# joelle-o-world/dusp

Measured on AMD Instinct MI355X. Metric: rendered Msamples/sec (whole node) + HBM GB/s fraction, 1024-voice 48kHz, higher is better.
Workload: dtype f64; 1 GPU; configs[2] per-voice: 1024 voices/GPU x Multiply(Osc(10k), Ramp(T,1,0) triggered), 60s @48000 Hz, every voice's PCM written; voices_per_gpu=1024, voices_total=1024, n_samples=2880000, engine=fused, parallelism=voices sharded over 1 GPU(s), no collective

## Files before the change

### dusp_amd/csrc/device_util.hpp

```cpp
#pragma once
#if !defined(__HIPCC_RTC__)
#include <hip/hip_runtime.h>
#endif

#include "device_types.hpp"
#include "filter_lamda.hpp"

namespace dusp {
namespace {

__device__ __forceinline__ int lsb_exponent(double x) {
    int ex;
    const double fr = frexp(fabs(x), &ex);
    const long long m = (long long)ldexp(fr, 53);
    return ex - 53 + __builtin_ctzll((unsigned long long)m);
}
__device__ __forceinline__ uint64_t addmod(uint64_t a, uint64_t b, uint64_t S) {
    const uint64_t s = a + b;
    return s >= S ? s - S : s;
}
__device__ __forceinline__ uint64_t mulmod(uint64_t a, uint64_t n, uint64_t S) {
    uint64_t acc = 0;
    for (int bit = 63 - __builtin_clzll(n | 1); bit >= 0; --bit) {
        acc = addmod(acc, acc, S);
        if ((n >> bit) & 1) acc = addmod(acc, a, S);
    }
    return acc;
}

__device__ __forceinline__ float operand_value(const DevOperand &o, const float *params, uint32_t n_inst, uint32_t inst) {
    return o.kind == SRC_PARAM ? params[(size_t)o.idx * n_inst + inst] : o.cval;
}

enum : int { TABLE_FORM_DATA = 0, TABLE_FORM_SAW = 1, TABLE_FORM_SQUARE = 2, TABLE_FORM_TRIANGLE = 3, TABLE_FORM_8BIT = 4 };

#if defined(__HIPCC__) || defined(__HIPCC_RTC__)
#define DUSP_HD __host__ __device__ __forceinline__
#else
#define DUSP_HD inline
#endif

struct TableForm {
    int32_t form;
    uint32_t sr, half, quarter;
    double N, rcp_N, srd, rcp_sr;
};

DUSP_HD TableForm make_table_form(int form, uint32_t sample_rate) {
    TableForm F;
    F.form = form;
    F.sr = sample_rate;
    F.half = sample_rate / 2;
    F.quarter = sample_rate / 4;
    F.N = (double)sample_rate + 1.0;
    F.rcp_N = 1.0 / F.N;
    F.srd = (double)sample_rate;
    F.rcp_sr = 1.0 / F.srd;
    return F;
}

DUSP_HD double refined_quotient(double x, double d, double rcp) {
    const double q = x * rcp;
    return fma(fma(-q, d, x), rcp, q);
}

DUSP_HD double js_round_small(double x) {
    const double r = floor(x + 0.5);
    return (r == 0.0 && (x < 0.0 || (x == 0.0 && 1.0 / x < 0.0))) ? -0.0 : r;
}

DUSP_HD float closed_table_entry(const TableForm &F, uint32_t i) {
    if (F.form == TABLE_FORM_SQUARE) return i < F.half ? 1.f : -1.f;
    if (i >= F.sr) return 0.f;
    if (F.form == TABLE_FORM_SAW) return (float)(-1.0 + refined_quotient((double)(2u * i), F.N, F.rcp_N));
    const uint32_t seg = (i >= F.quarter ? 1u : 0u) + (i >= 2u * F.quarter ? 1u : 0u) + (i >= 3u * F.quarter ? 1u : 0u);
    const float base = (float)(refined_quotient((double)(i - seg * F.quarter), F.srd, F.rcp_sr) * 4.0);
    return seg == 0 ? base : seg == 1 ? (float)(1.0 - (double)base) : seg == 2 ? -base : (float)(-1.0 + (double)base);
}
DUSP_HD float eightbit_of_sine(float sine) { return (float)(js_round_small((double)sine * 128.0) / 128.0); }

__device__ __forceinline__ uint32_t abs_diff(uint32_t a, uint32_t b) {
    uint32_t r;
    asm("v_sad_u32 %0, %1, %2, 0" : "=v"(r) : "v"(a), "s"(b));
    return r;
}

template <int TBL>
struct Table {
    const float *g;
    const float *h;
    uint32_t N, M;
    TableForm form;
    __device__ __forceinline__ const float *word(uint32_t k) const {
        return (const float *)((const char *)h + ((k + (k >> 5)) << 2));
    }
    __device__ __forceinline__ float at(uint32_t i) const {
        if (TBL == 0) return g[i];
        if (TBL == 2) return closed_table_entry(form, i);
        const bool upper = i > M;
        const float v = *word(abs_diff(i, M) + (upper ? 0u : 1u));
        const float s = upper ? -v : v;
        return TBL == 3 ? eightbit_of_sine(s) : s;
    }
    __device__ __forceinline__ void pair(uint32_t i, float &a, float &b) const {
        if (TBL == 0) {
            a = g[i];
            b = g[i + 1];
            return;
        }
        if (TBL == 2) {
            a = closed_table_entry(form, i);
            b = closed_table_entry(form, i + 1 <= form.sr ? i + 1 : form.sr);
            return;
        }
        if (TBL == 3) {
            a = at(i);
            b = at(i + 1 < N ? i + 1 : N - 1);
            return;
        }
        const bool upper = i > M;
        const float *p = word(abs_diff(i, M));
        const float p0 = p[0], p1 = p[1];
        a = upper ? -p0 : p1;
        b = upper ? -p1 : p0;
    }
    template <bool D32>
    __device__ __forceinline__ void pair_delta_at(uint32_t a_img, bool upper, double &a, double &d) const {
        const float *p = word(a_img);
        const float p0 = p[0], p1 = p[1];
        a = (double)(upper ? -p0 : p1);
        delta<D32>(p0, p1, d);
    }
    template <bool D32>
    __device__ __forceinline__ void pair_delta(uint32_t i, double &a, double &d) const {
        if (TBL == 0) {
            const float x = g[i], y = g[i + 1];
            a = (double)x;
            delta<D32>(y, x, d);
        } else
            pair_delta_at<D32>(abs_diff(i, M), i > M, a, d);
    }
    template <bool D32>
    static __device__ __forceinline__ void delta(float y, float x, double &d) {
        if (D32) {
            float df;
            asm("v_sub_f32 %0, %1, %2" : "=v"(df) : "v"(y), "v"(x));
            d = (double)df;
        } else
            d = (double)y - (double)x;
    }
};

__device__ __forceinline__ float lerp_delta(double a, double d, uint32_t F) {
    return (float)fma(d, (double)F * (1.0 / 4294967296.0), a);
}

constexpr uint32_t kPhaseBias = 0x41300000u;
struct LeanPhase {
    template <bool WRAPPED>
    static __device__ __forceinline__ void locate(unsigned long long Pc, uint32_t sr, uint32_t M, uint32_t &a_img, bool &upper, double &fraction) {
        const uint32_t h = (uint32_t)(Pc >> 32);
        if (WRAPPED) {
            a_img = abs_diff(h, kPhaseBias + M);
            upper = h > kPhaseBias + M;
        } else {
            const uint32_t s = abs_diff(h, kPhaseBias + sr);
            a_img = abs_diff(s, M);
            upper = (s > M) != (h < kPhaseBias + sr);
        }
        fraction = __builtin_amdgcn_fract(__longlong_as_double((long long)Pc));
    }
    static __device__ __forceinline__ uint32_t index(unsigned long long Pc, uint32_t sr) {
        const uint32_t h = (uint32_t)(Pc >> 32);
        return min(h - kPhaseBias, h - (kPhaseBias + sr));
    }
    static __device__ __forceinline__ unsigned long long step(unsigned long long P, unsigned long long c, uint32_t sr) {
        const unsigned long long s = P + c;
        const uint32_t h = (uint32_t)(s >> 32);
        const uint32_t u = h - sr;
        return ((unsigned long long)(u >= kPhaseBias ? u : h) << 32) | (uint32_t)s;
    }
};

__device__ __forceinline__ uint32_t mod_u32(uint32_t x, uint32_t m, double inv_m) {
    const uint32_t q = (uint32_t)((double)x * inv_m);
    uint32_t r = x - q * m;
    if ((int32_t)r < 0) r += m;
    if (r >= m) r -= m;
    return r;
}
__device__ __forceinline__ uint64_t mod_u64(uint64_t x, uint64_t m, double inv_m) {
    const uint64_t q = (uint64_t)((double)x * inv_m);
    uint64_t r = x - q * m;
    if ((int64_t)r < 0) r += m;
    if ((int64_t)r < 0) r += m;
    if (r >= m) r -= m;
    if (r >= m) r -= m;
    return r;
}

__device__ __forceinline__ unsigned long long mod_u64_lifted(unsigned long long x, unsigned long long m, double inv_m) {
    return mod_u64(x, m, inv_m);
}

template <bool FINITE>
__device__ __forceinline__ float fix_out(float v) {
    if (FINITE) return v + 0.f;
    return __builtin_amdgcn_classf(v, 0x23) ? 0.f : v;
}

template <bool VEC>
__device__ __forceinline__ void store4(float *row, const float (&v)[4], uint64_t t, uint64_t n_samples) {
    if (VEC) {
#ifdef DUSP_NT_STORES
        __builtin_nontemporal_store(f32x4{v[0], v[1], v[2], v[3]}, (f32x4 *)row);
#else
        *(f32x4 *)row = f32x4{v[0], v[1], v[2], v[3]};
#endif
    } else
        for (int c = 0; c < 4; ++c)
            if (t + c < n_samples) row[c] = v[c];
}

template <int BLOCK>
__device__ __forceinline__ void load_half_table(float *lds, const float *table, uint32_t sample_rate) {
    const uint32_t last = sample_rate / 2 + 1;
    const uint32_t n_words = last + (last >> 5) + 2;
    for (uint32_t q = threadIdx.x; q < n_words; q += BLOCK) {
        const uint32_t t = (q / 33) * 32 + (q % 33);
        lds[q] = table[last - min(t, last)];
    }
    __syncthreads();
}

__host__ __device__ inline size_t half_table_lds_bytes(uint32_t sample_rate) { return (size_t)half_table_image_bytes(sample_rate); }

}
}
```

### dusp_amd/csrc/fused_engine.hip

```cpp
#include <hip/hip_runtime.h>

#include <type_traits>

#include "device_types.hpp"
#include "fused_device.hpp"
#include "fused_plan.hpp"
#include "repeat_add.hpp"

namespace dusp {

namespace {

template <bool FASTDIV>
__device__ __forceinline__ float ramp_value(const FusedArgs &A, double tn, double dy) {
    const double tt = fmin(tn, A.r_d);
    double q;
    if (FASTDIV) {
        q = tt * A.r_rcp;
        const double rem = fma(-q, A.r_d, tt);
        q = fma(rem, A.r_rcp, q);
    } else
        q = tt / A.r_d;
    return (float)(A.r_y0 + q * dy);
}

__device__ __forceinline__ float shape_value(const FusedArgs &A, double t, double srd) {
    const double l = (double)A.s_min, h = (double)A.s_max;
    if (t <= 0.0) return (float)((A.s_left_is_shape ? (double)A.s_table[0] : A.s_left) * (h - l) + l);
    if (t > srd) return (float)((A.s_right_is_shape ? (double)A.s_table[(uint32_t)srd] : A.s_right) * (h - l) + l);
    if (t != t) return __builtin_nanf("");
    const double fl = floor(t), frac = t - fl;
    return (float)(l + (h - l) * ((double)A.s_table[(int)ceil(t)] * frac + (double)A.s_table[(int)fl] * (1.0 - frac)));
}

__device__ __forceinline__ void start_phase(const OscRec &rc, uint32_t seg, uint32_t lane, uint64_t (&P)[4]) {
    const uint64_t base = addmod(addmod(rc.P0, rc.Fm, rc.S), mulmod(rc.segstep, seg, rc.S), rc.S);
    P[0] = addmod(base, mulmod(rc.step4, lane, rc.S), rc.S);
    for (int c = 1; c < 4; ++c) P[c] = addmod(P[c - 1], rc.Fm, rc.S);
}

}

__global__ void dusp_fused_prepare(FusedArgs A, OscRec *recs) {
    const uint32_t inst = blockIdx.x * blockDim.x + threadIdx.x;
    if (inst >= A.n_inst) return;
    const uint32_t sr = A.sample_rate;
    const double srd = (double)sr;
    OscRec rc;
    double fd = (double)operand_value(A.f, A.params, A.n_inst, inst);
    rc.bad = !(fabs(fd) <= 3.0e38);
    if (rc.bad) fd = 0.0;
    if (fabs(fd) >= srd) fd = fmod(fd, srd);
    int E = 0;
    if (fd != 0.0) E = min(E, lsb_exponent(fd));
    if (A.phase0 != 0.0) E = min(E, lsb_exponent(A.phase0));
    const int Emin = -(62 - (32 - __builtin_clz(sr)));
    if (E < Emin) E = Emin;
    rc.E = E;
    rc.u = ldexp(1.0, E);
    rc.S = (uint64_t)sr << (-E);
    const long long F = (long long)rint(ldexp(fd, -E));
    rc.Fm = F >= 0 ? (uint64_t)F : rc.S - (uint64_t)(-F);
    if (rc.Fm >= rc.S) rc.Fm -= rc.S;
    rc.P0 = (uint64_t)rint(ldexp(A.phase0, -E));
    if (rc.P0 >= rc.S) rc.P0 %= rc.S;
    rc.step4 = mulmod(rc.Fm, 4, rc.S);
    rc.step256 = mulmod(rc.Fm, kChunk, rc.S);
    rc.segstep = mulmod(rc.Fm, (uint64_t)A.seg_groups * kChunk, rc.S);
    rc.gain = A.gain.kind == SRC_PARAM || A.gain.kind == SRC_CONST ? operand_value(A.gain, A.params, A.n_inst, inst) : 1.f;
    rc.pad = 0;
    recs[inst] = rc;

    const uint64_t T_end = (uint64_t)A.n_chunks * kChunk;
    double phase_end = (double)addmod(rc.P0, mulmod(rc.Fm, T_end, rc.S), rc.S) * rc.u;
    if (rc.bad) phase_end = __builtin_nan("");
    A.end_state[(size_t)A.osc_state_word * A.n_inst + inst] = phase_end;
    if (A.ramp_state_word >= 0) {
        const double t_end = A.r_playing ? fmin(A.r_t0 + (double)T_end, A.r_d) : A.r_t0;
        const bool playing_end = A.r_playing && (A.r_t0 + (double)T_end <= A.r_d);
        A.end_state[(size_t)A.ramp_state_word * A.n_inst + inst] = t_end;
        A.end_state[(size_t)(A.ramp_state_word + 1) * A.n_inst + inst] = playing_end ? 1.0 : 0.0;
    }
    if (A.shape_state_word >= 0) {
        const double t_end = A.s_playing ? repeat_add(A.s_t0, A.s_c, T_end) : A.s_t0;
        A.end_state[(size_t)A.shape_state_word * A.n_inst + inst] = t_end;
        A.end_state[(size_t)(A.shape_state_word + 1) * A.n_inst + inst] = A.s_playing ? 1.0 : 0.0;
        A.end_state[(size_t)(A.shape_state_word + 2) * A.n_inst + inst] = (A.s_finished || (T_end > 0 && t_end > srd)) ? 1.0 : 0.0;
    }
}

template <int KIND, int TBL, int R, bool FASTDIV, bool FINITE, int BLOCK>
__global__ void __launch_bounds__(BLOCK) dusp_fused_kernel(FusedArgs A, const OscRec *__restrict__ recs) {
    extern __shared__ __attribute__((aligned(16))) float lds_table[];
    Table<TBL> table;
    table.g = A.table;
    table.h = lds_table;
    table.N = A.sample_rate + 1;
    table.M = A.sample_rate / 2;
    table.form = make_table_form(A.table_form, A.sample_rate);
    if (TBL == 1) load_half_table<BLOCK>(lds_table, A.table, A.sample_rate);
    const uint32_t lane = threadIdx.x & 63u;
    constexpr uint32_t waves_per_block = BLOCK / 64;
    constexpr int RS = R < 4 ? R : 4;
    const uint32_t n_blk = (A.n_inst + R - 1) / R;
    const uint64_t n_items = (uint64_t)n_blk * A.n_seg;
    const uint64_t total_waves = (uint64_t)gridDim.x * waves_per_block;
    const double srd = (double)A.sample_rate;
    const uint32_t sr = A.sample_rate;
    const double dy = A.r_y1 - A.r_y0;
    const uint32_t n_full = A.vec4_ok ? (uint32_t)(A.n_samples / kChunk) : 0u;

    for (uint64_t item = (uint64_t)blockIdx.x * waves_per_block + (threadIdx.x >> 6); item < n_items; item += total_waves) {
        const uint32_t blk = A.seg_major ? (uint32_t)(item / A.n_seg) : (uint32_t)(item % n_blk);
        const uint32_t seg = A.seg_major ? (uint32_t)(item % A.n_seg) : (uint32_t)(item / n_blk);
        const uint32_t g0 = seg * A.seg_groups;
        const uint32_t g1 = min(g0 + A.seg_groups, A.n_groups);
        const uint32_t gm = max(g0, min(g1, n_full));
        const uint64_t t_start = (uint64_t)g0 * kChunk;

        uint32_t inst[R];
        int e_min = 0;
        bool any_bad = false;
#pragma unroll
        for (int r = 0; r < R; ++r) {
            inst[r] = min(blk * R + r, A.n_inst - 1);
            e_min = min(e_min, recs[inst[r]].E);
            any_bad = any_bad || recs[inst[r]].bad;
        }
        float *const row0 = A.out + t_start + lane * 4;
        const double tn0 = A.r_t0 + (A.r_playing ? (double)(t_start + lane * 4 + 1) : 0.0);
        const double tn_step = A.r_playing ? (double)kChunk : 0.0;
        const double tn_c = A.r_playing ? 1.0 : 0.0;
        double tn;
        const double st0 = (KIND == FUSED_OSC_SHAPE && A.s_playing) ? repeat_add(A.s_t0, A.s_c, t_start) : A.s_t0;
        double st;
        auto ramp4 = [&](float (&rv)[4]) {
            if (KIND == FUSED_OSC_SHAPE) {
                if (!A.s_playing) {
#pragma unroll
                    for (int c = 0; c < 4; ++c) rv[c] = shape_value(A, st, srd);
                } else {
                    long long T, ce;
                    int K;
                    if (linear_run(st, A.s_c, kChunk, T, ce, K)) {
                        T += (long long)(lane * 4) * ce;
#pragma unroll
                        for (int c = 0; c < 4; ++c) {
                            T += ce;
                            rv[c] = shape_value(A, ldexp((double)T, K - 52), srd);
                        }
                        st = ldexp((double)(T + (long long)(kChunk - 4 - lane * 4) * ce), K - 52);
                    } else {
                        double t = repeat_add(st, A.s_c, (uint64_t)lane * 4);
#pragma unroll
                        for (int c = 0; c < 4; ++c) rv[c] = shape_value(A, t = t + A.s_c, srd);
                        st = __shfl(t, 63, 64);
                    }
                }
            }
            if (KIND == FUSED_OSC_RAMP) {
                rv[0] = ramp_value<FASTDIV>(A, tn, dy);
#pragma unroll
                for (int c = 1; c < 4; ++c) rv[c] = ramp_value<FASTDIV>(A, tn + tn_c * c, dy);
                tn += tn_step;
            }
        };
        auto finish = [&](float v, float rv, float gain) {
            if (KIND == FUSED_OSC_RAMP || KIND == FUSED_OSC_SHAPE) v = v * rv;
            if (KIND == FUSED_OSC_GAIN) v = v * gain;
            return fix_out<FINITE>(v);
        };

        if (e_min == 0 && !any_bad) {
            uint32_t idx[R][4], step[R];
            size_t roff[R];
            float gain[R];
#pragma unroll
            for (int r = 0; r < R; ++r) {
                const OscRec rc = recs[inst[r]];
                uint64_t P[4];
                start_phase(rc, seg, lane, P);
                for (int c = 0; c < 4; ++c) idx[r][c] = (uint32_t)P[c];
                step[r] = (uint32_t)rc.step256;
                roff[r] = (size_t)inst[r] * A.n_samples;
                gain[r] = rc.gain;
            }
            tn = tn0;
            st = st0;
            float *row = row0;
            auto run = [&](uint32_t ga, uint32_t gb, auto vec) {
                for (uint32_t g = ga; g < gb; ++g) {
                    float rv[4] = {1.f, 1.f, 1.f, 1.f};
                    ramp4(rv);
#pragma unroll
                    for (int r = 0; r < R; ++r) {
                        float v[4];
#pragma unroll
                        for (int c = 0; c < 4; ++c) {
                            v[c] = finish(table.at(idx[r][c]), rv[c], gain[r]);
                            idx[r][c] += step[r];
                            idx[r][c] = min(idx[r][c], idx[r][c] - sr);
                        }
                        store4<decltype(vec)::value>(row + roff[r], v, (uint64_t)g * kChunk + lane * 4, A.n_samples);
                    }
                    row += kChunk;
                }
            };
            run(g0, gm, std::true_type{});
            run(gm, g1, std::false_type{});
        } else if (e_min >= -32 && !any_bad && A.fx32_ok) {
            for (int sub = 0; sub < R; sub += RS) {
                uint32_t I[RS][4], F[RS][4], dI[RS], dF[RS];
                size_t roff[RS];
                float gain[RS];
#pragma unroll
                for (int r = 0; r < RS; ++r) {
                    const OscRec rc = recs[inst[sub + r]];
                    const int sh = -rc.E;
                    uint64_t P[4];
                    start_phase(rc, seg, lane, P);
                    for (int c = 0; c < 4; ++c) {
                        I[r][c] = (uint32_t)(P[c] >> sh);
                        F[r][c] = sh ? (uint32_t)(P[c] << (32 - sh)) : 0u;
                    }
                    dI[r] = (uint32_t)(rc.step256 >> sh);
                    dF[r] = sh ? (uint32_t)(rc.step256 << (32 - sh)) : 0u;
                    roff[r] = (size_t)inst[sub + r] * A.n_samples;
                    gain[r] = rc.gain;
                }
                tn = tn0;
            st = st0;
                float *row = row0;
                if ((TBL == 0 || TBL == 1) && e_min >= -28 && A.table_delta) {
                    unsigned long long PD[RS], Q1[RS], Q2[RS], Q3[RS], C[RS];
                    auto uni = [](unsigned long long v) {
                        return ((unsigned long long)(uint32_t)__builtin_amdgcn_readfirstlane((int)(uint32_t)(v >> 32)) << 32) | (uint32_t)__builtin_amdgcn_readfirstlane((int)(uint32_t)v);
                    };
#pragma unroll
                    for (int r = 0; r < RS; ++r) {
                        const OscRec rc = recs[inst[sub + r]];
                        const int up = 32 + rc.E;
                        PD[r] = (((unsigned long long)(I[r][0] + kPhaseBias)) << 32) | F[r][0];
                        const uint64_t q2 = addmod(rc.Fm, rc.Fm, rc.S);
                        Q1[r] = uni(rc.Fm << up);
                        Q2[r] = uni(q2 << up);
                        Q3[r] = uni(addmod(q2, rc.Fm, rc.S) << up);
                        C[r] = uni(rc.step256 << up);
                    }
                    auto run_delta = [&](uint32_t ga, uint32_t gb, auto vec, auto d32) {
                        for (uint32_t g = ga; g < gb; ++g) {
                            float rv[4] = {1.f, 1.f, 1.f, 1.f};
                            ramp4(rv);
#pragma unroll
                            for (int r = 0; r < RS; ++r) {
                                float v[4];
                                double ta[4], td[4], fr[4];
#pragma unroll
                                for (int c = 0; c < 4; ++c) {
                                    const unsigned long long Pc = c == 0 ? PD[r] : PD[r] + (c == 1 ? Q1[r] : c == 2 ? Q2[r] : Q3[r]);
                                    if (TBL == 1) {
                                        uint32_t a_img;
                                        bool upper;
                                        if (c == 0) LeanPhase::locate<true>(Pc, sr, table.M, a_img, upper, fr[c]);
                                        else LeanPhase::locate<false>(Pc, sr, table.M, a_img, upper, fr[c]);
                                        table.template pair_delta_at<decltype(d32)::value>(a_img, upper, ta[c], td[c]);
                                    } else {
                                        fr[c] = __builtin_amdgcn_fract(__longlong_as_double((long long)Pc));
                                        table.template pair_delta<decltype(d32)::value>(LeanPhase::index(Pc, sr), ta[c], td[c]);
                                    }
                                }
#pragma unroll
                                for (int c = 0; c < 4; ++c) v[c] = finish((float)fma(td[c], fr[c], ta[c]), rv[c], gain[r]);
                                PD[r] = LeanPhase::step(PD[r], C[r], sr);
                                store4<decltype(vec)::value>(row + roff[r], v, (uint64_t)g * kChunk + lane * 4, A.n_samples);
                            }
                            row += kChunk;
                        }
                    };
                    if (A.table_delta == 2) {
                        run_delta(g0, gm, std::true_type{}, std::true_type{});
                        run_delta(gm, g1, std::false_type{}, std::true_type{});
                    } else {
                        run_delta(g0, gm, std::true_type{}, std::false_type{});
                        run_delta(gm, g1, std::false_type{}, std::false_type{});
                    }
                    continue;
                }
                const bool lean = KIND == FUSED_OSC_RAMP && FINITE && e_min >= -28 && A.r_scale_ok;
                auto run_lean = [&](uint32_t ga, uint32_t gb, auto vec) {
                    typedef float f32x2 __attribute__((ext_vector_type(2)));
                    for (uint32_t g = ga; g < gb; ++g) {
                        float rv[4] = {1.f, 1.f, 1.f, 1.f};
                        ramp4(rv);
                        const f32x2 e01 = f32x2{ldexpf(rv[0], -32), ldexpf(rv[1], -32)}, e23 = f32x2{ldexpf(rv[2], -32), ldexpf(rv[3], -32)};
#pragma unroll
                        for (int r = 0; r < RS; ++r) {
                            float x[4];
#pragma unroll
                            for (int c = 0; c < 4; ++c) {
                                float ta, tb;
                                table.pair(I[r][c], ta, tb);
                                const double wb = (double)F[r][c];
                                const double wa = 4294967296.0 - wb;
                                x[c] = (float)fma((double)tb, wb, (double)ta * wa);
                                const uint32_t f2 = F[r][c] + dF[r];
                                uint32_t i2 = I[r][c] + dI[r] + (f2 < F[r][c] ? 1u : 0u);
                                i2 = min(i2, i2 - sr);
                                F[r][c] = f2;
                                I[r][c] = i2;
                            }
                            const f32x2 zero = f32x2{0.f, 0.f};
                            const f32x2 p01 = f32x2{x[0], x[1]} * e01 + zero, p23 = f32x2{x[2], x[3]} * e23 + zero;
                            const float v[4] = {p01[0], p01[1], p23[0], p23[1]};
                            store4<decltype(vec)::value>(row + roff[r], v, (uint64_t)g * kChunk + lane * 4, A.n_samples);
                        }
                        row += kChunk;
                    }
                };
                if (lean) {
                    run_lean(g0, gm, std::true_type{});
                    run_lean(gm, g1, std::false_type{});
                    continue;
                }
                auto run = [&](uint32_t ga, uint32_t gb, auto vec) {
                    for (uint32_t g = ga; g < gb; ++g) {
                        float rv[4] = {1.f, 1.f, 1.f, 1.f};
                        ramp4(rv);
#pragma unroll
                        for (int r = 0; r < RS; ++r) {
                            float v[4];
#pragma unroll
                            for (int c = 0; c < 4; ++c) {
                                float ta, tb;
                                table.pair(I[r][c], ta, tb);
                                const double wb = (double)F[r][c];
                                const double wa = 4294967296.0 - wb;
                                const float x = (float)((double)ta * wa + (double)tb * wb);
                                v[c] = finish(ldexpf(x, -32), rv[c], gain[r]);
                                const uint32_t f2 = F[r][c] + dF[r];
                                uint32_t i2 = I[r][c] + dI[r] + (f2 < F[r][c] ? 1u : 0u);
                                i2 = min(i2, i2 - sr);
                                F[r][c] = f2;
                                I[r][c] = i2;
                            }
                            store4<decltype(vec)::value>(row + roff[r], v, (uint64_t)g * kChunk + lane * 4, A.n_samples);
                        }
                        row += kChunk;
                    }
                };
                run(g0, gm, std::true_type{});
                run(gm, g1, std::false_type{});
            }
        } else {
            for (int sub = 0; sub < R; sub += RS) {
                double ph[RS][4], D[RS];
                size_t roff[RS];
                float gain[RS];
                bool bad[RS];
#pragma unroll
                for (int r = 0; r < RS; ++r) {
                    const OscRec rc = recs[inst[sub + r]];
                    uint64_t P[4];
                    start_phase(rc, seg, lane, P);
                    for (int c = 0; c < 4; ++c) ph[r][c] = (double)P[c] * rc.u;
                    D[r] = (double)rc.step256 * rc.u;
                    roff[r] = (size_t)inst[sub + r] * A.n_samples;
                    gain[r] = rc.gain;
                    bad[r] = rc.bad;
                }
                tn = tn0;
            st = st0;
                float *row = row0;
                auto run = [&](uint32_t ga, uint32_t gb, auto vec) {
                    for (uint32_t g = ga; g < gb; ++g) {
                        float rv[4] = {1.f, 1.f, 1.f, 1.f};
                        ramp4(rv);
#pragma unroll
                        for (int r = 0; r < RS; ++r) {
                            float v[4];
#pragma unroll
                            for (int c = 0; c < 4; ++c) {
                                const uint32_t idx = (uint32_t)(int)ph[r][c];
                                const double fraction = ph[r][c] - (double)(int)idx;
                                float ta, tb;
                                table.pair(idx, ta, tb);
                                float x = (float)((double)ta * (1.0 - fraction) + (double)tb * fraction);
                                if (bad[r]) x = 0.f;
                                v[c] = finish(x, rv[c], gain[r]);
                                ph[r][c] += D[r];
                                if (ph[r][c] >= srd) ph[r][c] -= srd;
                            }
                            store4<decltype(vec)::value>(row + roff[r], v, (uint64_t)g * kChunk + lane * 4, A.n_samples);
                        }
                        row += kChunk;
                    }
                };
                run(g0, gm, std::true_type{});
                run(gm, g1, std::false_type{});
            }
        }
    }
}

template <int KIND, int TBL, int R, bool FASTDIV, bool FINITE, int BLOCK>
static hipError_t launch_one(const FusedArgs &A, const OscRec *recs, int grid, size_t lds_bytes, hipStream_t stream) {
    auto kernel = dusp_fused_kernel<KIND, TBL, R, FASTDIV, FINITE, BLOCK>;
    if (lds_bytes > 65536) {
        hipError_t e = hipFuncSetAttribute((const void *)kernel, hipFuncAttributeMaxDynamicSharedMemorySize, (int)lds_bytes);
        if (e != hipSuccess) return e;
    }
    hipLaunchKernelGGL(kernel, dim3((unsigned)grid), dim3(BLOCK), lds_bytes, stream, A, recs);
    return hipGetLastError();
}

hipError_t launch_fused(const FusedPlan &plan, const FusedLaunch &L, hipStream_t stream) {
    FusedArgs A{};
    A.params = L.params;
    A.table = L.tables + (size_t)plan.table_id * L.table_stride;
    A.out = L.out;
    A.end_state = L.end_state;
    A.n_samples = L.n_samples;
    A.n_inst = L.n_inst;
    A.n_groups = (uint32_t)((L.n_samples + kChunk - 1) / kChunk);
    A.sample_rate = L.sample_rate;
    A.n_chunks = L.n_chunks;
    A.f = plan.f;
    A.gain = plan.gain;
    if (plan.kind != FUSED_OSC_GAIN) A.gain.kind = -1;
    A.phase0 = plan.phase0;
    A.r_d = plan.r_d; A.r_y0 = plan.r_y0; A.r_y1 = plan.r_y1; A.r_t0 = plan.r_t0; A.r_rcp = plan.r_rcp;
    A.r_playing = plan.r_playing;
    A.r_fastdiv = plan.r_fastdiv;
    A.vec4_ok = (L.n_samples % 4 == 0) && (((uintptr_t)L.out & 15) == 0);
    A.osc_state_word = 0;
    A.ramp_state_word = plan.kind == FUSED_OSC_RAMP ? 1 : -1;
    A.shape_state_word = plan.kind == FUSED_OSC_SHAPE ? 1 : -1;
    if (plan.kind == FUSED_OSC_SHAPE) {
        A.s_table = L.tables + (size_t)plan.s_table_id * L.table_stride;
        A.s_t0 = plan.s_t0; A.s_c = plan.s_c; A.s_min = plan.s_min; A.s_max = plan.s_max;
        A.s_left = plan.s_left; A.s_right = plan.s_right;
        A.s_left_is_shape = plan.s_left_is_shape; A.s_right_is_shape = plan.s_right_is_shape;
        A.s_playing = plan.s_playing; A.s_finished = plan.s_finished;
    }
    auto ordinary = [](double y) { return y == 0.0 || (std::fabs(y) >= 9.3e-10 && std::fabs(y) <= 1.1e18); };
    A.r_scale_ok = plan.kind == FUSED_OSC_RAMP && ordinary(plan.r_y0) && ordinary(plan.r_y1) && plan.r_d <= 1.1e12 && (plan.r_t0 == 0.0 || plan.r_t0 >= 1.0) &&
                           L.knobs.fused_fx32 != 2
                       ? 1 : 0;
    A.fx32_ok = L.table_fx32_ok && L.knobs.fused_fx32 ? 1 : 0;
    A.table_delta = L.knobs.fused_fx32 == 1 ? L.table_delta : 0;
    A.seg_major = L.knobs.fused_segmajor;

    int tbl = (L.table_antisym && L.sample_rate % 2 == 0) ? 1 : 0;
    if (L.table_form >= TABLE_FORM_SAW && L.table_form <= TABLE_FORM_TRIANGLE) tbl = 2;
    A.table_form = L.table_form;
    if (L.knobs.fused_table_global) tbl = 0;
    const size_t lds_bytes = tbl == 1 ? half_table_lds_bytes(L.sample_rate) : 0;
    if (lds_bytes > 160 * 1024) tbl = 0;

    int R = L.knobs.fused_R;
    if (R != 1 && R != 4 && R != 8) R = 4;
    const int block = tbl == 1 ? 1024 : 256;
    const int grid = tbl == 1 ? L.n_cus : L.n_cus * 8;
    const uint64_t total_waves = (uint64_t)grid * (block / 64);
    const uint64_t n_blk = (A.n_inst + R - 1) / R;
    auto cut = [&](uint64_t per_wave, uint64_t &n_seg) {
        n_seg = std::max<uint64_t>(1, (total_waves * per_wave + n_blk - 1) / n_blk);
        return (A.n_groups + n_seg - 1) / n_seg;
    };
    uint64_t n_seg = 1, seg = 0;
    if (L.knobs.fused_items > 0) seg = cut((uint64_t)L.knobs.fused_items, n_seg);
    else if ((seg = cut(4, n_seg)) < 64) seg = cut(2, n_seg);
    if (seg < 16) seg = 16;
    if (seg > 4096) seg = 4096;
    A.seg_groups = (uint32_t)seg;
    A.n_seg = (A.n_groups + A.seg_groups - 1) / A.seg_groups;
    const bool finite = L.table_finite && plan.kind != FUSED_OSC_GAIN && std::isfinite(plan.r_y0) && std::isfinite(plan.r_y1);

    hipLaunchKernelGGL(dusp_fused_prepare, dim3((A.n_inst + 255) / 256), dim3(256), 0, stream, A, L.recs);
    hipError_t e = hipGetLastError();
    if (e != hipSuccess) return e;

#define DUSP_L3(KIND, RR, FD, FIN) \
    return tbl == 1 ? launch_one<KIND, 1, RR, FD, FIN, 1024>(A, L.recs, grid, lds_bytes, stream) \
                    : launch_one<KIND, 0, RR, FD, FIN, 256>(A, L.recs, grid, 0, stream)
#define DUSP_L2(KIND, FD, FIN) \
    do { if (tbl == 2) return launch_one<KIND, 2, 4, FD, FIN, 256>(A, L.recs, grid, 0, stream); \
         if (R == 8) { DUSP_L3(KIND, 8, FD, FIN); } if (R == 4) { DUSP_L3(KIND, 4, FD, FIN); } DUSP_L3(KIND, 1, FD, FIN); } while (0)
    switch (plan.kind) {
    case FUSED_OSC:
        if (finite) DUSP_L2(FUSED_OSC, false, true);
        DUSP_L2(FUSED_OSC, false, false);
    case FUSED_OSC_RAMP:
        if (plan.r_fastdiv && finite) DUSP_L2(FUSED_OSC_RAMP, true, true);
        if (plan.r_fastdiv) DUSP_L2(FUSED_OSC_RAMP, true, false);
        DUSP_L2(FUSED_OSC_RAMP, false, false);
    case FUSED_OSC_GAIN: DUSP_L2(FUSED_OSC_GAIN, false, false);
    case FUSED_OSC_SHAPE: DUSP_L2(FUSED_OSC_SHAPE, false, false);
    }
#undef DUSP_L2
#undef DUSP_L3
    return hipErrorInvalidValue;
}

}
```

### dusp_amd/csrc/fused_plan.hpp

```cpp
#pragma once
#include <cmath>
#include <string>
#include <vector>

#include "device_types.hpp"
#include "program.hpp"

namespace dusp {

enum : int { FUSED_OSC = 0, FUSED_OSC_RAMP = 1, FUSED_OSC_GAIN = 2, FUSED_SUMCHAIN = 3, FUSED_OSC_SHAPE = 4 };

struct FusedPlan {
    std::string shape, why;
    int kind = FUSED_OSC;
    int table_id = 0;
    DevOperand f{}, gain{};
    double phase0 = 0;
    double r_d = 1, r_y0 = 0, r_y1 = 0, r_t0 = 0, r_rcp = 1;
    int r_playing = 0, r_fastdiv = 0;
    int s_table_id = 0, s_playing = 0, s_finished = 0, s_left_is_shape = 0, s_right_is_shape = 0;
    double s_t0 = 0, s_c = 0, s_left = 0, s_right = 0;
    float s_min = 0, s_max = 1;
    std::vector<double> sum_f, sum_phase0;
    std::vector<int> sum_units;
    bool sum_all_int = false;
    int sum_env = 0;
    std::vector<float> sum_gain;
    std::vector<int> sum_ramp_units;
    int n_state_words = 0;
    std::vector<int> unit_state_first, unit_state_count;
};

struct OscRec {
    uint64_t S, Fm, P0;
    uint64_t step4, step256, segstep;
    double u;
    int32_t E, bad;
    float gain, pad;
};

struct SumVoice {
    uint64_t B0, bs, step4, step256, Fm;
    float gain;
    uint32_t pad;
};

struct SumArgs {
    const SumVoice *voices;
    const float *table;
    float *out;
    uint64_t n_samples, S;
    double inv_S, inv_sr;
    uint32_t n_voices, n_inst, n_groups, n_blocks, sample_rate, vec4_ok;
    double r_d, r_y0, r_y1, r_t0;
    int32_t r_playing, r_fastdiv;
    const float *init;
    uint32_t first_block, raw;
};

struct WaveArgs {
    const DevOp *ops;
    const int32_t *out_bufs;
    const float *params;
    const float *tables;
    float *out;
    double *state;
    const double *init_state;
    uint64_t n_samples;
    uint32_t n_ops, n_out, n_inst, n_pad, n_bufs, n_groups, sample_rate, table_stride, vec4_ok;
    int32_t lds_table_id;
    uint32_t table_bytes, wave_bytes;
    float *rings;
    uint64_t ring_samples, clock0;
    uint32_t has_filter, scratch_bytes;
    const float *inputs;
    uint32_t n_state_ops;
    uint32_t ring_events;
    uint32_t ext_units;
    uint32_t n_seg, seg_groups;
    uint32_t pass_mode;
    uint32_t pass_level;
    unsigned long long *seg_sum, *seg_start;
    int32_t max_osc_level, pad4;
    float *saved_bufs;
    uint32_t save_bufs, resume;
    uint32_t n_params, param_bytes;
};

inline size_t wave_param_bytes(size_t n_params) { return n_params && n_params <= 2048 ? (n_params * 4 + 15) & ~(size_t)15 : 0; }
inline size_t wave_lds_bytes(size_t n_bufs, size_t n_state_ops, size_t scratch_bytes) {
    return (n_bufs * 1024 + n_state_ops * 96 + (scratch_bytes ? scratch_bytes + 16 : 0) + 15) & ~(size_t)15;
}

struct WavePlan {
    bool ok = false, has_filter = false;
    int scratch_bytes = 0;
    std::vector<int> order;
    std::vector<int> buf_slot;
    std::vector<int> op_state;
    int n_slots = 0, n_state_ops = 0;
    int ext_units = 0;
    bool ring_events = false;
    bool splittable = false;
    bool splittable_but_for_filters = false;
    int max_osc_level = 0;
    std::vector<int> osc_level;
    std::vector<int> ramp_fastdiv;
    struct RampChecked { double d, t0; bool ok; };
    std::vector<RampChecked> ramp_checked;
    int lds_table_id = -1;
    std::string why;
};

struct FusedLaunch {
    const float *params;
    const float *tables;
    float *out;
    double *end_state;
    OscRec *recs;
    uint64_t n_samples;
    uint32_t n_inst, n_chunks, sample_rate, table_stride;
    int n_cus;
    bool table_antisym, table_finite, table_fx32_ok;
    const float *chain_init = nullptr;
    uint64_t chain_first = 0;
    bool chain_raw = false;
    int table_delta;
    int table_form;
    Knobs knobs;
};

struct FusedArgs {
    const float *params;
    const float *table;
    float *out;
    double *end_state;
    uint64_t n_samples;
    uint32_t n_inst, n_groups, seg_groups, n_seg, sample_rate, n_chunks;
    DevOperand f, gain;
    double phase0;
    double r_d, r_y0, r_y1, r_t0, r_rcp;
    int32_t r_playing, r_fastdiv, vec4_ok, osc_state_word, ramp_state_word, fx32_ok, seg_major, r_scale_ok;
    const float *s_table;
    double s_t0, s_c, s_left, s_right;
    float s_min, s_max;
    int32_t s_playing, s_finished, shape_state_word, s_left_is_shape, s_right_is_shape;
    int32_t table_form;
    int32_t table_delta;
};

inline bool ramp_fastdiv_ok(double t0, double d, bool playing) {
    const double r = 1.0 / d;
    auto same = [&](double t) {
        const double q = t * r;
        const double rem = std::fma(-q, d, t);
        return std::fma(rem, r, q) == t / d;
    };
    if (!same(t0) || !same(d)) return false;
    if (!playing) return true;
    const double steps = std::ceil(d - t0) + 1;
    if (!(steps < 67108864.0)) return false;
    double t = t0;
    for (long k = 0; k < (long)steps; k++) {
        t += 1.0;
        if (t > d) break;
        if (!same(t)) return false;
    }
    return true;
}

inline bool plan_fused(const Program &P, FusedPlan &plan) {
    const Graph &g = P.g;
    auto no = [&](const std::string &why) {
        plan.why = why;
        return false;
    };
    if (!P.warm_ops.empty()) return no("channel counts grow during the first chunks");
    if (!P.feed_forward) return no("feedback edge");
    if (!g.rings.empty() || P.ring_samples) return no("rings");
    if (P.out_bufs.size() != 1) return no("multichannel output");
    for (const auto &u : g.units)
        if (u.n_out != 1) return no("multichannel unit");

    std::vector<int> used(g.units.size(), 0);
    int osc_unit = -1, ramp_unit = -1, shape_unit = -1;
    bool have_gain = false;
    auto leaf_k = [&](const InletDesc &in) { return in.kind != IN_CONNECT && in.vals.size() == 1; };
    auto take_osc = [&](int ui) {
        const UnitDesc &u = g.units[(size_t)ui];
        if (u.op != OP_OSC || !leaf_k(u.inlets[0]) || osc_unit >= 0) return false;
        osc_unit = ui;
        used[(size_t)ui]++;
        return true;
    };
    const UnitDesc &root = g.units[(size_t)g.out_unit];
    used[(size_t)g.out_unit]++;
    if (root.op == OP_OSC) {
        used[(size_t)g.out_unit]--;
        if (!take_osc(g.out_unit)) return no("Osc with a connected f");
        plan.kind = FUSED_OSC;
        plan.shape = "osc(k)";
    } else if (root.op == OP_MULTIPLY) {
        for (int k = 0; k < 2; k++) {
            const InletDesc &in = root.inlets[(size_t)k];
            if (in.kind == IN_CONNECT) {
                const UnitDesc &s = g.units[(size_t)in.src_unit];
                if (s.op == OP_OSC) {
                    if (!take_osc(in.src_unit)) return no("second Osc / connected f");
                } else if (s.op == OP_RAMP && ramp_unit < 0 && shape_unit < 0) {
                    ramp_unit = in.src_unit;
                    used[(size_t)in.src_unit]++;
                } else if (s.op == OP_SHAPE && ramp_unit < 0 && shape_unit < 0) {
                    shape_unit = in.src_unit;
                    used[(size_t)in.src_unit]++;
                } else
                    return no("unsupported Multiply operand");
            } else if (leaf_k(in) && !have_gain) {
                have_gain = true;
                plan.gain = make_operand(g, in, 0);
            } else
                return no("unsupported Multiply operand");
        }
        if (osc_unit < 0) return no("no Osc under Multiply");
        if (ramp_unit >= 0) {
            plan.kind = FUSED_OSC_RAMP;
            plan.shape = "mul(osc(k),ramp)";
        } else if (shape_unit >= 0) {
            plan.kind = FUSED_OSC_SHAPE;
            plan.shape = "mul(osc(k),shape)";
        } else if (have_gain) {
            plan.kind = FUSED_OSC_GAIN;
            plan.shape = "mul(osc(k),k)";
        } else
            return no("Multiply of two Oscs");
    } else if (root.op == OP_SUM) {
        std::vector<int> rev;
        int cur = g.out_unit;
        for (;;) {
            const UnitDesc &su = g.units[(size_t)cur];
            int next = -1, oscs[2] = {-1, -1};
            for (int k = 0; k < 2; k++) {
                const InletDesc &in = su.inlets[(size_t)k];
                if (in.kind != IN_CONNECT) return no("Sum with a constant operand");
                const UnitDesc &s = g.units[(size_t)in.src_unit];
                if (s.op == OP_SUM && next < 0) next = in.src_unit;
                else if (s.op == OP_OSC || s.op == OP_MULTIPLY) oscs[k] = in.src_unit;
                else return no("unsupported Sum operand");
            }
            if (next >= 0) {
                rev.push_back(oscs[0] >= 0 ? oscs[0] : oscs[1]);
                used[(size_t)next]++;
                cur = next;
            } else {
                rev.push_back(oscs[1]);
                rev.push_back(oscs[0]);
                break;
            }
            if (rev.size() > 70000) return no("chain too long");
        }
        plan.kind = FUSED_SUMCHAIN;
        plan.shape = "sumchain(osc(k) x " + std::to_string(rev.size()) + ")";
        plan.sum_all_int = true;
        plan.sum_env = -1;
        for (auto it = rev.rbegin(); it != rev.rend(); ++it) {
            int ui = *it;
            if (ui < 0) return no("malformed chain");
            int env = 0;
            if (g.units[(size_t)ui].op == OP_MULTIPLY) {
                const UnitDesc &m = g.units[(size_t)ui];
                used[(size_t)ui]++;
                int osc = -1;
                for (int k = 0; k < 2; k++) {
                    const InletDesc &in = m.inlets[(size_t)k];
                    if (in.kind == IN_CONNECT && g.units[(size_t)in.src_unit].op == OP_OSC && osc < 0) osc = in.src_unit;
                    else if (in.kind == IN_CONNECT && g.units[(size_t)in.src_unit].op == OP_RAMP && env == 0) {
                        env = 2;
                        const UnitDesc &r = g.units[(size_t)in.src_unit];
                        used[(size_t)in.src_unit]++;
                        if (plan.sum_ramp_units.empty()) {
                            plan.r_d = r.attrs[0]; plan.r_y0 = r.attrs[1]; plan.r_y1 = r.attrs[2];
                            plan.r_t0 = r.state[0]; plan.r_playing = r.state[1] != 0;
                        } else if (plan.r_d != r.attrs[0] || plan.r_y0 != r.attrs[1] || plan.r_y1 != r.attrs[2] || plan.r_t0 != r.state[0] ||
                                   plan.r_playing != (r.state[1] != 0))
                            return no("chain voices with different Ramps");
                        plan.sum_ramp_units.push_back(in.src_unit);
                    } else if (in.kind == IN_CONST && in.vals.size() == 1 && env == 0) {
                        env = 1;
                        plan.sum_gain.push_back((float)in.vals[0]);
                    } else
                        return no("unsupported voice in the chain");
                }
                if (osc < 0 || env == 0) return no("unsupported voice in the chain");
                ui = osc;
            }
            if (plan.sum_env < 0) plan.sum_env = env;
            else if (plan.sum_env != env) return no("chain voices of different kinds");
            const UnitDesc &o = g.units[(size_t)ui];
            if (o.op != OP_OSC) return no("malformed chain");
            used[(size_t)ui]++;
            const InletDesc &fin = o.inlets[0];
            if (fin.kind != IN_CONST || fin.vals.size() != 1) return no("chain oscillator needs a constant f");
            const double f = (double)(float)fin.vals[0];
            if (!std::isfinite(f)) return no("non-finite f");
            const double fr = std::fmod(f, (double)g.sample_rate), p0 = o.state[0];
            if (std::ldexp(fr, 32) != std::floor(std::ldexp(fr, 32))) return no("f finer than 2^-32");
            if (!(p0 >= 0 && p0 < g.sample_rate) || std::ldexp(p0, 32) != std::floor(std::ldexp(p0, 32)))
                return no("start phase not on the 2^-32 grid");
            if (fr != std::floor(fr) || p0 != std::floor(p0)) plan.sum_all_int = false;
            if (plan.sum_units.empty()) plan.table_id = (int)o.attrs[0];
            else if (plan.table_id != (int)o.attrs[0]) return no("mixed waveforms");
            plan.sum_units.push_back(ui);
            plan.sum_f.push_back(fr);
            plan.sum_phase0.push_back(p0);
        }
        for (size_t i = 0; i < used.size(); i++)
            if (used[i] != 1) return no("circuit has units outside the fused tree");
        plan.unit_state_first.assign(g.units.size(), 0);
        plan.unit_state_count.assign(g.units.size(), 0);
        plan.n_state_words = 0;
        for (int ui : plan.sum_units) {
            plan.unit_state_first[(size_t)ui] = plan.n_state_words++;
            plan.unit_state_count[(size_t)ui] = 1;
        }
        if (plan.sum_env == 2) {
            if (!(plan.r_d > 0) || !std::isfinite(plan.r_d) || !std::isfinite(plan.r_t0) || plan.r_t0 > plan.r_d || (plan.r_playing && !(plan.r_t0 + 1 >= 0)))
                return no("chain Ramp outside the closed-form regime");
            plan.r_rcp = 1.0 / plan.r_d;
            plan.r_fastdiv = ramp_fastdiv_ok(plan.r_t0, plan.r_d, plan.r_playing != 0) ? 1 : 0;
            for (int ui : plan.sum_ramp_units) {
                plan.unit_state_first[(size_t)ui] = plan.n_state_words;
                plan.unit_state_count[(size_t)ui] = 2;
                plan.n_state_words += 2;
            }
        }
        if (plan.sum_env == 1) plan.shape = "sumchain(osc(k) * k x " + std::to_string(plan.sum_units.size()) + ")";
        if (plan.sum_env == 2) plan.shape = "sumchain(osc(k) * ramp x " + std::to_string(plan.sum_units.size()) + ")";
        return true;
    } else
        return no("root is not an Osc, a Multiply or a Sum chain");
    for (size_t i = 0; i < used.size(); i++)
        if (used[i] != 1) return no("circuit has units outside the fused tree");

    const UnitDesc &osc = g.units[(size_t)osc_unit];
    plan.table_id = (int)osc.attrs[0];
    plan.f = make_operand(g, osc.inlets[0], 0);
    plan.phase0 = osc.state[0];
    if (!(plan.phase0 >= 0 && plan.phase0 < g.sample_rate)) return no("Osc phase outside [0, sampleRate)");
    {
        const double scaled = std::ldexp(plan.phase0, 36);
        if (scaled != std::floor(scaled)) return no("Osc start phase finer than 2^-36");
    }
    if (ramp_unit >= 0) {
        const UnitDesc &r = g.units[(size_t)ramp_unit];
        plan.r_d = r.attrs[0];
        plan.r_y0 = r.attrs[1];
        plan.r_y1 = r.attrs[2];
        plan.r_t0 = r.state[0];
        plan.r_playing = r.state[1] != 0;
        if (!(plan.r_d > 0) || !std::isfinite(plan.r_d) || !std::isfinite(plan.r_t0)) return no("degenerate Ramp duration");
        if (plan.r_playing && !(plan.r_t0 + 1 >= 0)) return no("Ramp starts below -1");
        if (plan.r_t0 > plan.r_d) return no("Ramp starts past its end");
        plan.r_rcp = 1.0 / plan.r_d;
        plan.r_fastdiv = ramp_fastdiv_ok(plan.r_t0, plan.r_d, plan.r_playing != 0) ? 1 : 0;
    }
    if (shape_unit >= 0) {
        const UnitDesc &sh = g.units[(size_t)shape_unit];
        for (int k = 0; k < 3; k++)
            if (sh.inlets[(size_t)k].kind != IN_CONST || sh.inlets[(size_t)k].vals.size() != 1) return no("Shape with a connected / per-instance inlet");
        plan.s_table_id = (int)sh.attrs[0];
        plan.s_left_is_shape = sh.attrs[1] != 0;
        plan.s_left = sh.attrs[2];
        plan.s_right_is_shape = sh.attrs[3] != 0;
        plan.s_right = sh.attrs[4];
        plan.s_t0 = sh.state[0];
        plan.s_playing = sh.state[1] != 0;
        plan.s_finished = sh.state[2] != 0;
        plan.s_c = 1.0 / (double)(float)sh.inlets[0].vals[0];
        plan.s_min = (float)sh.inlets[1].vals[0];
        plan.s_max = (float)sh.inlets[2].vals[0];
        if (plan.s_playing && !(plan.s_t0 >= 0 && plan.s_c > 0 && plan.s_c < 1e300)) return no("Shape outside the closed-form regime");
        if (!std::isfinite(plan.s_t0)) return no("Shape with a non-finite t");
    }
    plan.unit_state_first.assign(g.units.size(), 0);
    plan.unit_state_count.assign(g.units.size(), 0);
    plan.n_state_words = 0;
    plan.unit_state_first[(size_t)osc_unit] = plan.n_state_words;
    plan.unit_state_count[(size_t)osc_unit] = 1;
    plan.n_state_words += 1;
    if (ramp_unit >= 0) {
        plan.unit_state_first[(size_t)ramp_unit] = plan.n_state_words;
        plan.unit_state_count[(size_t)ramp_unit] = 2;
        plan.n_state_words += 2;
    }
    if (shape_unit >= 0) {
        plan.unit_state_first[(size_t)shape_unit] = plan.n_state_words;
        plan.unit_state_count[(size_t)shape_unit] = 3;
        plan.n_state_words += 3;
    }
    return true;
}

inline void build_sum_voices(const FusedPlan &plan, uint32_t sample_rate, int gb, uint64_t T_end, std::vector<SumVoice> &voices,
                             std::vector<double> &end_phase) {
    typedef unsigned __int128 u128;
    const uint64_t S = (uint64_t)sample_rate << 32;
    voices.clear();
    end_phase.clear();
    for (size_t j = 0; j < plan.sum_f.size(); j++) {
        const double f = plan.sum_f[j];
        const long long F = (long long)std::ldexp(f, 32);
        const uint64_t Fm = F >= 0 ? (uint64_t)F % S : (S - (uint64_t)(-F) % S) % S;
        const uint64_t P0 = (uint64_t)std::ldexp(plan.sum_phase0[j], 32);
        SumVoice v;
        v.Fm = Fm;
        v.B0 = (uint64_t)(((u128)P0 + Fm) % S);
        v.bs = (uint64_t)(((u128)Fm * (uint64_t)(gb * kChunk)) % S);
        v.step4 = (uint64_t)(((u128)Fm * 4) % S);
        v.step256 = (uint64_t)(((u128)Fm * kChunk) % S);
        v.gain = plan.sum_env == 1 ? plan.sum_gain[j] : 1.f;
        v.pad = 0;
        voices.push_back(v);
        end_phase.push_back(std::ldexp((double)(uint64_t)(((u128)P0 + (u128)Fm * T_end) % S), -32));
    }
    if (plan.sum_env == 2)
        for (size_t j = 0; j < plan.sum_ramp_units.size(); j++) {
            const double since = (double)T_end;
            end_phase.push_back(plan.r_playing ? std::fmin(plan.r_t0 + since, plan.r_d) : plan.r_t0);
            end_phase.push_back((plan.r_playing && plan.r_t0 + since <= plan.r_d) ? 1.0 : 0.0);
        }
}

enum : int { DELAY_REGIME_UNKNOWN = 0, DELAY_REGIME_LONG = 1, DELAY_REGIME_SHORT = 2, DELAY_REGIME_OTHER = 4 };
#if defined(__HIPCC__)
__host__ __device__
#endif
inline int delay_value_regime(float delay, int64_t ring_len, bool mono) {
    double d = (double)delay;
    if (!(d >= 0.0) || !(d < 4.0e9)) return DELAY_REGIME_OTHER;
    const double len = (double)ring_len;
    if (d >= (mono ? 0.0 : 1.0) && d < (double)(kChunk - 1) && ring_len >= 2 * kChunk) return DELAY_REGIME_SHORT;
    if (d >= len) d = fmod(d, len);
    const double fl = floor(d);
    if (fl >= (double)kChunk && fl + (double)kChunk <= len) return DELAY_REGIME_LONG;
    return DELAY_REGIME_OTHER;
}

inline bool delay_write_once(const DevOp &op) {
    if (op.in[1].kind == SRC_PARAM) return op.in[1].pad == DELAY_REGIME_LONG;
    if (op.in[1].kind != SRC_CONST) return false;
    const double len = (double)op.ring_len;
    double dconst = (double)op.in[1].cval;
// ... 221 lines not shown
```

Before: 1.317 million Msamples/s.

## Add LDS half-table fast path with folded byte-address phase and fused envelope multiply

Adds a dedicated path for the antisymmetric half-sine LDS table. The phase is tracked directly as a biased byte address, so each lookup becomes one sad plus a shift-add to form the padded LDS address, and the wrap is handled by a min. When the ramp scale and fx32 conditions allow, it also multiplies the table value by the envelope with a plain fmaf instead of the generic finish routine. This cuts integer ALU work per sample in a kernel that may be store-bound, at the risk of exactness differences if the fma shortcut does not match finish().

```diff
diff --git a/dusp_amd/csrc/device_util.hpp b/dusp_amd/csrc/device_util.hpp
--- a/dusp_amd/csrc/device_util.hpp
+++ b/dusp_amd/csrc/device_util.hpp
@@ -83,6 +83,13 @@
     uint32_t r;
     asm("v_sad_u32 %0, %1, %2, 0" : "=v"(r) : "v"(a), "s"(b));
     return r;
+}
+
+__device__ __forceinline__ uint32_t half_image_byte(uint32_t u, uint32_t C) {
+    const uint32_t b = max(u, C) - min(u, C) + 2u;
+    uint32_t a;
+    asm("v_lshl_add_u32 %0, %1, 2, %2" : "=v"(a) : "v"(b >> 7), "v"(b));
+    return a;
 }
 
 template <int TBL>
diff --git a/dusp_amd/csrc/fused_engine.hip b/dusp_amd/csrc/fused_engine.hip
--- a/dusp_amd/csrc/fused_engine.hip
+++ b/dusp_amd/csrc/fused_engine.hip
@@ -171,7 +171,59 @@
             return fix_out<FINITE>(v);
         };
 
-        if (e_min == 0 && !any_bad) {
+        if (TBL == 1 && e_min == 0 && !any_bad) {
+            uint32_t u[R][4], du[R];
+            size_t roff[R];
+            float gain[R];
+#pragma unroll
+            for (int r = 0; r < R; ++r) {
+                const OscRec rc = recs[inst[r]];
+                uint64_t P[4];
+                start_phase(rc, seg, lane, P);
+                for (int c = 0; c < 4; ++c) u[r][c] = 4u * (uint32_t)P[c] + 2u;
+                du[r] = 4u * (uint32_t)rc.step256;
+                roff[r] = (size_t)inst[r] * A.n_samples;
+                gain[r] = rc.gain;
+            }
+            const uint32_t C = 2u * sr + 4u, W = 4u * sr;
+            tn = tn0;
+            st = st0;
+            float *row = row0;
+            auto run = [&](uint32_t ga, uint32_t gb, auto vec, auto fma_env) {
+                for (uint32_t g = ga; g < gb; ++g) {
+                    float e[R][4];
+#pragma unroll
+                    for (int r = 0; r < R; ++r)
+#pragma unroll
+                        for (int c = 0; c < 4; ++c)
+                            e[r][c] = *(const __attribute__((address_space(3))) float *)(uintptr_t)half_image_byte(u[r][c], C);
+                    __builtin_amdgcn_sched_barrier(0);
+                    float rv[4] = {1.f, 1.f, 1.f, 1.f};
+                    ramp4(rv);
+#pragma unroll
+                    for (int r = 0; r < R; ++r) {
+                        float v[4];
+#pragma unroll
+                        for (int c = 0; c < 4; ++c) {
+                            const float t = u[r][c] > C ? -e[r][c] : e[r][c];
+                            v[c] = decltype(fma_env)::value ? __builtin_fmaf(t, rv[c], 0.f) : finish(t, rv[c], gain[r]);
+                            u[r][c] += du[r];
+                            u[r][c] = min(u[r][c], u[r][c] - W);
+                        }
+                        store4<decltype(vec)::value>(row + roff[r], v, (uint64_t)g * kChunk + lane * 4, A.n_samples);
+                    }
+                    row += kChunk;
+                }
+            };
+            constexpr bool may_fma = KIND == FUSED_OSC_RAMP && FINITE;
+            if (may_fma && A.env_fma) {
+                run(g0, gm, std::true_type{}, std::integral_constant<bool, may_fma>{});
+                run(gm, g1, std::false_type{}, std::integral_constant<bool, may_fma>{});
+            } else {
+                run(g0, gm, std::true_type{}, std::false_type{});
+                run(gm, g1, std::false_type{}, std::false_type{});
+            }
+        } else if (e_min == 0 && !any_bad) {
             uint32_t idx[R][4], step[R];
             size_t roff[R];
             float gain[R];
@@ -449,6 +501,7 @@
     A.fx32_ok = L.table_fx32_ok && L.knobs.fused_fx32 ? 1 : 0;
     A.table_delta = L.knobs.fused_fx32 == 1 ? L.table_delta : 0;
     A.seg_major = L.knobs.fused_segmajor;
+    A.env_fma = A.r_scale_ok && L.table_fx32_ok ? 1 : 0;
 
     int tbl = (L.table_antisym && L.sample_rate % 2 == 0) ? 1 : 0;
     if (L.table_form >= TABLE_FORM_SAW && L.table_form <= TABLE_FORM_TRIANGLE) tbl = 2;
diff --git a/dusp_amd/csrc/fused_plan.hpp b/dusp_amd/csrc/fused_plan.hpp
--- a/dusp_amd/csrc/fused_plan.hpp
+++ b/dusp_amd/csrc/fused_plan.hpp
@@ -147,6 +147,7 @@
     int32_t s_playing, s_finished, shape_state_word, s_left_is_shape, s_right_is_shape;
     int32_t table_form;
     int32_t table_delta;
+    int32_t env_fma;
 };
 
 inline bool ramp_fastdiv_ok(double t0, double d, bool playing) {
```

Measured after the change: 1.330 million Msamples/s, median of 6. 1.01x the previous value.
